# kgnlp/allophant

Measured on AMD Instinct MI355X. Metric: encoder frames/sec (whole node), 10s x 32 utterances @16kHz, higher is better.
Workload: dtype f16x3

## Files before the change

allophant_amd/csrc/amx_api.hip:

```cpp
#include "../../include/allophant_amx.h"
#include "../../include/allophant_amx_allophones.h"
#include "../../include/allophant_amx_beam.h"
#include "../../include/allophant_amx_align.h"
#include "../../include/allophant_amx_score.h"
#include "../../include/allophant_amx_search.h"
#include "../../include/allophant_amx_resample.h"
#include "../../include/allophant_amx_edit.h"
#include "amx_common.h"

#include <algorithm>
#include <cmath>
#include <cstdio>
#include <cstring>
#include <initializer_list>
#include <map>
#include <cstdlib>
#include <string>
#include <vector>

using namespace amx;

namespace {

thread_local std::string g_create_error;
// ... 1106 lines not shown
struct PassPlan {
    uint32_t flags = 0;
    int N = 0;
    int64_t L = 0;
    const float* d_audio = nullptr;
    float* d_out = nullptr;
    int64_t total = 0;
    int NT = 2, prec = 0, C = 0, D = 0, F = 0, H = 0, dh = 64, dhp = 64, E = 0, Eld = 0, cg = 0;
    int64_t Ts[AMX_MAX_CONV + 1] = {};
    int T = 0, Tp = 0, TpTot = 0, Tpad = 0;
    int64_t M = 0, Mp = 0, Mrows = 0, Mh = 0, rows1 = 0, rows2 = 0, xp_plane = 0, qk_plane = 0;
    size_t qkv_bytes = 0;
    bool keep = false, masked = true, stable = true, blanks = true;
    bool packed = false, packed_early = false, ragged = false, window_ok = false, needs_qkv_zero = false;
    bool fold = false, stream_in_planes = false;
    void *d_len = nullptr, *d_frames = nullptr, *d_rowoff = nullptr, *d_partial = nullptr, *d_stats = nullptr, *actA = nullptr, *actB = nullptr,
         *preln = nullptr, *hbuf = nullptr, *xp = nullptr, *hg = nullptr, *qb = nullptr, *kb = nullptr, *vtb = nullptr, *ao = nullptr, *ff = nullptr,
         *hfin = nullptr, *logits = nullptr, *hpk = nullptr, *splitk = nullptr, *gn_partial = nullptr, *gn_scale = nullptr, *gn_shift = nullptr,
         *ebuf = nullptr, *cat = nullptr, *tl_x = nullptr, *tl_p = nullptr, *tl_qkv = nullptr, *ln_rowps = nullptr, *ln_coef = nullptr,
         *ln_partial = nullptr;
    const int* d_frames_enc = nullptr;
    int* d_tiles = nullptr;
    size_t tile_first[AMX_MAX_CONV + 1] = {};
    std::vector<float*> saved;
    float* conv_dbg = nullptr;
    float* hfin_rows = nullptr;
    float* stream = nullptr;
    std::vector<int> rowoff_host, frames_host;

    GemmParams with_ws(GemmParams g) const {
        g.splitk_ws = (float*)splitk;
        g.splitk_ws_elems = splitk ? (int64_t)(SPLITK_BYTES / 4) : 0;
        return g;
    }
    AttnParams attn_params() const {
// ... 37 lines not shown
        return with_ws(g);
    }
    GemmParams ffn2_params(amx_handle h, const Layer& ly) const {
        GemmParams g{};
        g.A = ff; g.a_plane = pln(h, Mrows * F); g.lda = F; g.rows_per_batch = Mrows;
        g.W = ly.w2; g.w_plane = pln(h, (int64_t)D * F); g.ldw = F;
        g.M = (int)Mrows; g.N = D; g.K = F;
        g.scale = ly.r_2; g.bias = ly.b2;
        g.residual = stream; g.ldr = D; g.out_f32 = stream; g.ldo = D;
        return with_ws(g);
    }
    GemmParams as_consumer(GemmParams g, const float* col_c) const {
        g.row_coef = (const float2*)ln_coef; g.col_c = col_c;
        return g;
    }
    GemmParams as_producer(GemmParams g, bool f32 = true) const {
        g.ln_partial = (float2*)ln_partial; g.ln_rowps = (const float4*)ln_rowps;
        g.out_p = xp; g.out_plane = xp_plane; g.ldp = D;
        if (stream_in_planes) {
            g.ln_res_planes = 1;
            g.residual = nullptr;
            if (!f32) g.out_f32 = nullptr;
        }
        return g;
    }
};

}

static int pin_reserve(amx_handle h, int N, hipStream_t s) {
    HIPCHK(h, hipStreamSynchronize(s));
    for (int i = 0; i < amx_handle_s::PIN_SLOTS; ++i) {
// ... 229 lines not shown
    }
    P.blanks = c.dependency_blanks != 0;
    if ((rc = plan_concat(h, P, s))) return rc;
    P.needs_qkv_zero = !P.packed && (h->last_N != N || h->last_T != P.T || h->qkv_dirty);
    P.Mrows = P.packed ? P.Mp : P.M;
    P.xp_plane = pln(h, P.Mrows * D);
    P.qk_plane = P.packed ? (int64_t)H * P.TpTot * P.dhp : (int64_t)N * H * P.Tp * P.dhp;
    P.stream = (float*)(P.packed ? P.hpk : P.hbuf);
    if (P.packed_early) {
        P.rowoff_host.assign(pin_rowoff, pin_rowoff + N);
        P.frames_host.assign(pin_frames, pin_frames + N);
    }
    P.stream_in_planes = NT == 2;
    if (P.stable && c.layers > 0 && D % 64 == 0 && D <= 2048) {
        WS("ln_rowps", (size_t)P.Mrows * 16, P.ln_rowps);
        WS("ln_coef", (size_t)P.Mrows * 8, P.ln_coef);
        WS("ln_partial", (size_t)P.Mrows * (D / 64) * 8, P.ln_partial);
        const Layer& ly = h->layers[0];
        const int prec = P.prec;
        P.fold = gemm_ln_fold_ok(prec, P.as_consumer(P.qkv_params(h, ly), ly.c_qkv)) &&
                 gemm_ln_fold_ok(prec, P.as_producer(P.oproj_params(h, ly), false)) &&
                 gemm_ln_fold_ok(prec, P.as_consumer(P.ffn1_params(h, ly), ly.c_1)) &&
                 gemm_ln_fold_ok(prec, P.as_producer(P.ffn2_params(h, ly), false)) &&
                 gemm_ln_fold_ok(prec, P.as_producer(P.ffn2_params(h, ly), true));
    }
    ++h->pass_counter;
    h->last_fold = P.fold;
    h->last_packed = P.packed_early ? 2 : (P.packed ? 1 : 0);
    h->last_attention = c.layers > 0 ? attention_form(P.attn_params()) : -1;
    h->last_rows = P.Mrows;
    h->last_graph = 0;
#undef WS
    return AMX_OK;
}

static int enqueue_pass(amx_handle h, const PassPlan& P, hipStream_t s) {
    const amx_config& c = h->cfg;
    const int prec = P.prec, N = P.N, C = P.C, D = P.D, T = P.T;
    const int64_t M = P.M, Mh = P.Mh;
// ... 153 lines not shown
            pending.splits = splits;
        }
        gemm(g);
    };
    auto stream_norm = [&](const float* gamma, const float* beta, int64_t rows, int64_t plane, float* out_ln) {
        Timed t_(h, AMX_KC_ROWNORM);
        if (pending.on) {
            launch_fixup_rownorm(prec, pending.g, pending.splits, gamma, beta, c.eps, P.xp, plane, D, out_ln, D, s);
            pending.on = false;
        } else {
            launch_rownorm(prec, (const float*)hbuf, D, rows, D, gamma, beta, 0, nullptr, nullptr, c.eps, 0.f, P.xp, plane, D, out_ln, D, s);
        }
    };
    float* const ln_inplace = P.stable ? nullptr : (float*)hbuf;
    if (!P.stable) stream_norm(h->fln_g, h->fln_b, P.Mrows, P.xp_plane, ln_inplace);
    const int* const fold_frames = P.packed || !P.masked ? nullptr : P.d_frames_enc;
    auto ln_finalize = [&]() {
        Timed t_(h, AMX_KC_ROWNORM);
        launch_ln_finalize((const float2*)P.ln_partial, D / 64, P.Mrows, c.eps, (float4*)P.ln_rowps, (float2*)P.ln_coef, fold_frames, T, s);
    };
    for (int l = 0; l < c.layers; ++l) {
        const Layer& ly = h->layers[l];
        if (P.fold) {
            if (l == 0) {
                Timed t_(h, AMX_KC_ROWNORM);
                launch_ln_rowprep(prec, (const float*)hbuf, D, P.Mrows, D, c.eps, P.xp, P.xp_plane, D, (float4*)P.ln_rowps, (float2*)P.ln_coef,
                                  fold_frames, T, s);
            }
        } else if (P.stable) {
            stream_norm(h->unit_g, h->zero_b, P.Mrows, P.xp_plane, nullptr);
        }
        if (P.saved[l]) {
            if (P.packed_early) {
                launch_copy(P.saved[l], hbuf, (size_t)P.Mp * D * 4, s);
            } else {
                launch_copy(P.saved[l], P.packed ? hpad : hbuf, (size_t)M * D * 4, s);
                if (P.packed) launch_pack_rows(P.saved[l], (float*)hbuf, (const int*)P.d_rowoff, (const int*)P.d_frames, N, T, D, true, s);
            }
        }
        gemm(P.fold ? P.as_consumer(P.qkv_params(h, ly), ly.c_qkv) : P.qkv_params(h, ly));
        {
            Timed t_(h, AMX_KC_ATTENTION);
            launch_attention(prec, P.attn_params(), s);
        }
        if (P.fold) {
            residual_gemm(P.as_producer(P.oproj_params(h, ly), false), false);
            ln_finalize();
        } else {
            residual_gemm(P.oproj_params(h, ly), true);
            if (P.stable) stream_norm(h->unit_g, h->zero_b, P.Mrows, P.xp_plane, nullptr);
            else stream_norm(ly.ln1_g, ly.ln1_b, P.Mrows, P.xp_plane, ln_inplace);
        }
        gemm(P.fold ? P.as_consumer(P.ffn1_params(h, ly), ly.c_1) : P.ffn1_params(h, ly));
        if (P.fold && (l + 1 < c.layers || P.stream_in_planes)) {
            const bool last = l + 1 == c.layers;
            residual_gemm(P.as_producer(P.ffn2_params(h, ly), last || P.saved[l + 1] != nullptr), false);
            if (!last) ln_finalize();
        } else {
            residual_gemm(P.ffn2_params(h, ly), !P.fold && !(P.packed && !P.packed_early && l == c.layers - 1));
        }
        if (!P.stable) stream_norm(ly.ln2_g, ly.ln2_b, P.Mrows, P.xp_plane, ln_inplace);
    }
    if (refused) return fail(h, AMX_EINVAL, "internal: an encoder product of the LayerNorm fold had no kernel for its plan and was not launched");
    if (P.packed && !P.packed_early) {
        { Timed t_(h, AMX_KC_OTHER); launch_pack_rows((const float*)hpad, (float*)P.hpk, (const int*)P.d_rowoff, (const int*)P.d_frames, N, T, D, true, s); }
        hbuf = hpad;
    }
    if (P.stable) {
        stream_norm(h->fln_g, h->fln_b, Mh, pln(h, Mh * D), (float*)P.hfin);
    } else if (P.keep) {
        launch_copy(P.hfin, hbuf, (size_t)Mh * D * 4, s);
    }
// ... 958 lines not shown
```

allophant_amd/csrc/amx_common.h:

```cpp
#pragma once
#include <hip/hip_runtime.h>
#include <stdint.h>
#include <string>
#include <type_traits>

struct amx_resample_geometry;
struct amx_resample_row;

namespace amx {

typedef _Float16 f16;
typedef __bf16 bf16;
typedef __attribute__((ext_vector_type(8))) _Float16 f16x8;
typedef __attribute__((ext_vector_type(8))) __bf16 bf16x8;
typedef __attribute__((ext_vector_type(4))) _Float16 f16x4;
typedef __attribute__((ext_vector_type(4))) __bf16 bf16x4;
typedef __attribute__((ext_vector_type(2))) _Float16 f16x2;
typedef __attribute__((ext_vector_type(2))) __bf16 bf16x2;
typedef __attribute__((ext_vector_type(2))) float f32x2;
typedef __attribute__((ext_vector_type(4))) float f32x4;
typedef __attribute__((ext_vector_type(16))) float f32x16;

enum Precision { PREC_BF16 = 0, PREC_F16 = 1, PREC_BF16X3 = 2, PREC_F16X3 = 3 };
inline int prec_planes(int p) { return p >= 2 ? 2 : 1; }
// ... 200 lines not shown
    float* splitk_ws;
    int64_t splitk_ws_elems;
    int splits;
    int64_t split_out;
    const int* tile_list;
    int n_tiles;
    int defer_fixup;
    int a_taps;
    int64_t a_tap_stride;
    unsigned long long* stamps;
    const float4* ln_rowps;
    float2* ln_partial;
    int ln_res_planes;
    const float2* row_coef;
    const float* col_c;
};

extern bool g_force_generic_gemm;
bool launch_gemm(int prec, const GemmParams& p, hipStream_t stream);
bool gemm_uses_pp(int prec, const GemmParams& p);
bool gemm_fuses_ln(int prec, const GemmParams& p);
int gemm_ln_tap_minor_slice(int prec, const GemmParams& p);
int gemm_planned_splits(int prec, const GemmParams& p);
bool fixup_rownorm_eligible(const GemmParams& p);
void launch_fixup_rownorm(int prec, const GemmParams& p, int splits, const float* gamma, const float* beta, float eps, void* out_p,
                          int64_t out_plane, int64_t ldp, float* out_ln, int64_t ldo_ln, hipStream_t stream);
bool gemm_ln_fold_ok(int prec, const GemmParams& p);
void launch_gemm_grouped(int prec, const GemmParams& p, int groups, hipStream_t stream);

struct AttnParams {
    const void* q;
// ... 217 lines not shown
```

allophant_amd/csrc/amx_gemm.hip:

```cpp
#include "amx_common.h"
#include <algorithm>
#include <cstdlib>
#include <type_traits>

namespace amx {

bool g_force_generic_gemm = false;

namespace {

#include "amx_gemm_tile.inc"
#include "amx_gemm_pp.inc"
#include "amx_gemm_ln.inc"

int device_cus() {
    static int per_device[MAX_DEVICES] = {};
    const int dev = current_device();
    int& cus = per_device[dev];
    if (!cus) {
        hipDeviceProp_t prop;
        if (hipGetDeviceProperties(&prop, dev) == hipSuccess) cus = prop.multiProcessorCount;
        if (cus <= 0) cus = 256;
        cus -= cus % 8;
        if (cus < 8) cus = 8;
// ... 238 lines not shown

enum class GemmKernel { LN, LN_IL, PP, DMA, TILE };

struct GemmRoute {
    GemmKernel kernel = GemmKernel::TILE;
    int mi = 0, ni = 0;
    int fold = 0;
    int shape = 0;
    int bn = 0;
    int splits = 1;
    bool launches = true;
};

GemmRoute gemm_route(int NT, const GemmParams& p) {
    GemmRoute r;
    r.fold = p.ln_partial ? 2 : p.row_coef ? 1 : 0;
    if (p.ln_gamma) {
        r.kernel = ln_uses_il(NT, p) ? GemmKernel::LN_IL : GemmKernel::LN;
        r.launches = ln_eligible(NT, p);
        return r;
    }
    if (!dma_preferred_shape(NT, p) && pp_eligible(NT, p)) {
        r.kernel = GemmKernel::PP;
        pp_plan(NT, p, &r.mi, &r.splits, &r.ni);
        r.launches = !(r.fold == 2 && r.ni != 4);
        return r;
    }
    r.launches = !r.fold;
    r.shape = dma_tile_shape(NT, p, 1);
    if (r.shape) {
        r.kernel = GemmKernel::DMA;
// ... 87 lines not shown
}

static GemmRoute product_route_of(int prec, GemmParams p) {
    p.ln_gamma = nullptr;
    return route_of(prec, p);
}

bool gemm_uses_pp(int prec, const GemmParams& p) { return product_route_of(prec, p).kernel == GemmKernel::PP; }

bool gemm_ln_fold_ok(int prec, const GemmParams& p_in) {
    const GemmParams p = with_vec_flag(p_in);
    const int NT = prec_planes(prec);
    const GemmRoute r = product_route_of(prec, p_in);
    if (!p.vec_ok || r.kernel != GemmKernel::PP || r.splits != 1) return false;
    if (p.ln_partial) {
        if (r.ni != 4 || p.N % 64 || p.N > 2048 || !p.out_p || !p.ln_rowps || p.act || p.mode || p.row_len || p.row_coef) return false;
        if (p.ln_res_planes ? NT != 2 : (!p.out_f32 || !p.residual)) return false;
        if (NT == 2 && (p.out_plane != PLANE_IL || p.ldp % 32)) return false;
        if (p.ldp % 8 || ((uintptr_t)p.out_p & 15) || ((uintptr_t)p.ln_partial & 7) || ((uintptr_t)p.ln_rowps & 15)) return false;
    }
    if (p.row_coef) {
        if (!p.col_c || ((uintptr_t)p.col_c & 15) || ((uintptr_t)p.row_coef & 7) || p.residual || p.row_len) return false;
        if (p.mode != 1 && (!p.out_p || p.out_f32)) return false;
    }
    return true;
}

int gemm_planned_splits(int prec, const GemmParams& p) { return route_of(prec, p).splits; }

bool fixup_rownorm_eligible(const GemmParams& p) {
    return p.splitk_ws && p.out_f32 && !p.out_p && p.act == 0 && p.mode == 0 && !p.row_len && !p.ln_gamma && p.N % 4 == 0 &&
           p.N <= 1024 && p.ldo % 4 == 0 && (!p.residual || p.ldr % 4 == 0) && !((uintptr_t)p.out_f32 & 15) &&
           !((uintptr_t)p.residual & 15) && !((uintptr_t)p.bias & 15) && p.zout == 0;
}

void launch_fixup_rownorm(int prec, const GemmParams& p, int splits, const float* gamma, const float* beta, float eps, void* out_p,
                          int64_t out_plane, int64_t ldp, float* out_ln, int64_t ldo_ln, hipStream_t stream) {
    AMX_DISPATCH(prec, (launch_fixup_rownorm_t<T16, NT>(p, splits, gamma, beta, eps, out_p, out_plane, ldp, out_ln, ldo_ln, stream)));
// ... 17 lines not shown
```

allophant_amd/csrc/amx_gemm_pp.inc:

```

namespace pp {
constexpr int BN = 256;
constexpr int EPI_WAVE = 32 * 64 * 4;
template <int MI, int NI = 4>
struct Ring {
    static constexpr int A_BYTES = MI * 32 * 128, W_BYTES = NI * 64 * 128, SLICE = A_BYTES + W_BYTES;
    static constexpr int NSL = MI == 8 ? 2 : 3, DIST = NSL - 1;
    static constexpr int EPI_BASE = DIST * SLICE;
    static constexpr int LDS_BYTES = (NSL * SLICE > EPI_BASE + 8 * EPI_WAVE) ? NSL * SLICE : EPI_BASE + 8 * EPI_WAVE;
};
constexpr int lds_bytes(int NT, int MI, int NI = 4) {
    return MI == 8 ? (NI == 4 ? Ring<8, 4>::LDS_BYTES : Ring<8, 3>::LDS_BYTES) : (NI == 4 ? Ring<4, 4>::LDS_BYTES : Ring<4, 3>::LDS_BYTES);
}
constexpr int epi_base(int NT, int MI, int NI = 4) {
    return MI == 8 ? (NI == 4 ? Ring<8, 4>::EPI_BASE : Ring<8, 3>::EPI_BASE) : (NI == 4 ? Ring<4, 4>::EPI_BASE : Ring<4, 3>::EPI_BASE);
}
__device__ __forceinline__ int es_idx(int row, int chunk) { return row * 64 + ((chunk ^ (row & 7)) << 2); }
}

__device__ __forceinline__ void mfma16_acc(f32x4& c, f16x8 a, f16x8 b) {
    asm volatile("v_mfma_f32_16x16x32_f16 %0, %1, %2, %0" : "+v"(c) : "v"(a), "v"(b));
}
__device__ __forceinline__ void mfma16_acc(f32x4& c, bf16x8 a, bf16x8 b) {
    asm volatile("v_mfma_f32_16x16x32_bf16 %0, %1, %2, %0" : "+v"(c) : "v"(a), "v"(b));
// ... 151 lines not shown
            const float4 pr = ps[j % SLOTS][i];
            float4 v = make_float4(fmaf(c[i][0], scale, b4.x), fmaf(c[i][1], scale, b4.y), fmaf(c[i][2], scale, b4.z),
                                   fmaf(c[i][3], scale, b4.w));
            float4 res = r[j % SLOTS][i];
            if (RESP) {
                const uint4 raw = __builtin_bit_cast(uint4, res);
                res = pp_planes_residual<T>(make_uint2(raw.x, raw.y), make_uint2(raw.z, raw.w), pr.x, pow2_reciprocal(pr.y));
            }
            v.x += res.x; v.y += res.y; v.z += res.z; v.w += res.w;
            if (optr) *(float4*)(optr + (int64_t)row * p.ldo) = v;
            pp_emit_row<T, NT>(v, make_float2(pr.z, pr.w), ch, true, part + (int64_t)row * nblk, pbase + (int64_t)row * prow, plane);
        }
    }
}

template <typename T, int NT, bool ACT, bool QK, int MI, bool FINISHED = false, int NI = 4, bool COEF = false>
__device__ __forceinline__ void pp_epilogue_p16(const GemmParams& p, f32x4 (&acc)[NI][MI], float* es, int lane, int mw, int nw) {
    typedef typename Vec8<T>::type V8;
    const int c8 = NI == 4 || (lane & 7) < 2 * NI ? (lane & 7) : (lane & 7) - 2 * NI, rs = lane >> 3;
    const int n = nw + c8 * 8;
    const float scale = FINISHED ? 1.f : p.scale;
    float4 b0 = make_float4(0.f, 0.f, 0.f, 0.f), b1 = b0;
    if (!FINISHED && p.bias) { b0 = *(const float4*)(p.bias + n); b1 = *(const float4*)(p.bias + n + 4); }
    float4 cc0 = make_float4(0.f, 0.f, 0.f, 0.f), cc1 = cc0;
    if (COEF) { cc0 = *(const float4*)(p.col_c + n); cc1 = *(const float4*)(p.col_c + n + 4); }
    const float2* coef = COEF ? p.row_coef + (mw + rs) : nullptr;
    T* base;
    int64_t row_stride, plane;
    int b = 0, t = 0;
    if (QK) {
        const int D = p.H * p.dh;
        const int which = n / D;
        const int rem = n - which * D;
        const int hh = rem / p.dh, d = rem - hh * p.dh;
        base = (T*)(which == 0 ? p.q : (which == 1 ? p.k : p.v)) + (int64_t)hh * p.Tp * p.dhp + d;
        row_stride = p.dhp;
        plane = p.qk_plane;
        b = (mw + rs) / p.T;
        t = (mw + rs) - b * p.T;
    } else {
        const bool o_il = plane_is_il<NT>(p.out_plane);
        base = (T*)p.out_p + pidx((int64_t)(mw + rs) * p.ldp + n, o_il);
        row_stride = p.ldp << (o_il ? 1 : 0);
        plane = p.out_plane;
    }
    float2 cf_all[MI / 2][4];
    if (COEF) {
#pragma unroll
        for (int q = 0; q < MI / 2; ++q)
#pragma unroll
            for (int i = 0; i < 4; ++i) cf_all[q][i] = coef[q * 32 + i * 8];
    }
#pragma unroll
    for (int q = 0; q < MI / 2; ++q) {
        float2 cf[4];
        if (COEF) {
#pragma unroll
            for (int i = 0; i < 4; ++i) cf[i] = cf_all[q][i];
        }
        pp_stage_round(es, acc, q, lane);
        f32x4 c[4][2];
#pragma unroll
        for (int i = 0; i < 4; ++i) {
            c[i][0] = *(const f32x4*)(es + pp::es_idx(i * 8 + rs, 2 * c8));
            c[i][1] = *(const f32x4*)(es + pp::es_idx(i * 8 + rs, 2 * c8 + 1));
        }
#pragma unroll
        for (int i = 0; i < 4; ++i) {
            float v[8];
            if (COEF) {
                const float as = cf[i].x * scale, bs = cf[i].y;
                v[0] = fmaf(c[i][0][0], as, fmaf(bs, cc0.x, b0.x)); v[1] = fmaf(c[i][0][1], as, fmaf(bs, cc0.y, b0.y));
                v[2] = fmaf(c[i][0][2], as, fmaf(bs, cc0.z, b0.z)); v[3] = fmaf(c[i][0][3], as, fmaf(bs, cc0.w, b0.w));
// ... 18 lines not shown
                t += 8;
                const bool wrap = t >= p.T;
                t -= wrap ? p.T : 0;
                b += wrap ? 1 : 0;
            } else {
                dst = base + (int64_t)(q * 32 + i * 8) * row_stride;
            }
            *(V8*)dst = hv.v;
            if (NT > 1) *(V8*)(dst + plane) = lv.v;
        }
    }
}

template <typename T, int NT, int MI, bool FINISHED = false, int NI = 4, int FOLD = 0>
__device__ __forceinline__ void pp_epilogue_generic(const GemmParams& p, f32x4 (&acc)[NI][MI], float* es, int lane, int mw, int nw,
                                                    float* out_f32) {
    typedef typename Vec4<T>::type V4;
    const int D = p.H * p.dh;
    const float scale = FINISHED ? 1.f : p.scale;
    const int ch = lane & 15, rq = (lane >> 4) * 8;
    const int n = nw + ch * 4;
    const bool n_ok = n < p.N && ch < NI * 4;
    float4 bias4 = make_float4(0.f, 0.f, 0.f, 0.f);
    if (!FINISHED && p.bias && n_ok) bias4 = *(const float4*)(p.bias + n);
    int64_t qk_col = 0;
    T* qk_base = nullptr;
    if (p.mode == 1 && n_ok) {
        const int which = n / D;
        const int rem = n - which * D;
        const int hh = rem / p.dh, d = rem - hh * p.dh;
        qk_base = (T*)(which == 0 ? p.q : (which == 1 ? p.k : p.v));
// ... 5 lines not shown
    if (FOLD == 1 && n_ok) colc4 = *(const float4*)(p.col_c + n);
    constexpr bool emit = NI == 4 && FOLD == 2;
#pragma unroll
    for (int q = 0; q < MI / 2; ++q) {
        pp_stage_round(es, acc, q, lane);
        int b = 0, t = 0;
        if (need_bt) {
            const int mfirst = mw + q * 32 + rq;
            b = mfirst / rt;
            t = mfirst - b * rt;
        }
#pragma unroll
        for (int i = 0; i < 8; ++i) {
            const int m = mw + q * 32 + rq + i;
            const f32x4 c = *(const f32x4*)(es + pp::es_idx(rq + i, ch));
            if constexpr (emit) {
                const bool ok = m < p.M;
                const int mc = ok ? m : p.M - 1;
                float4 v = make_float4(fmaf(c[0], scale, bias4.x), fmaf(c[1], scale, bias4.y), fmaf(c[2], scale, bias4.z),
                                       fmaf(c[3], scale, bias4.w));
                const float4 pr = p.ln_rowps[mc];
                T* pdst = (T*)p.out_p + pidx((int64_t)mc * p.ldp + n, NT == 2);
                const int64_t plane = NT == 2 ? PLANE_IL : 0;
                float4 rr = make_float4(0.f, 0.f, 0.f, 0.f);
                if constexpr (NT == 2) {
                    if (p.ln_res_planes) rr = pp_planes_residual<T>(*(const uint2*)pdst, *(const uint2*)(pdst + plane), pr.x, pow2_reciprocal(pr.y));
                    else if (p.residual) rr = *(const float4*)(p.residual + (int64_t)mc * p.ldr + n);
                } else if (p.residual) {
                    rr = *(const float4*)(p.residual + (int64_t)mc * p.ldr + n);
                }
                v.x += rr.x; v.y += rr.y; v.z += rr.z; v.w += rr.w;
                if (ok && out_f32) *(float4*)(out_f32 + (int64_t)m * p.ldo + n) = v;
                pp_emit_row<T, NT>(v, make_float2(pr.z, pr.w), ch, ok, p.ln_partial + (int64_t)mc * (p.N >> 6) + (n >> 6), pdst, plane);
                continue;
            }
            if (m < p.M && n_ok) {
                float v[4];
                if (FOLD == 1) {
                    const float2 cf = p.row_coef[m];
                    const float as = cf.x * scale;
                    v[0] = fmaf(c[0], as, fmaf(cf.y, colc4.x, bias4.x)); v[1] = fmaf(c[1], as, fmaf(cf.y, colc4.y, bias4.y));
                    v[2] = fmaf(c[2], as, fmaf(cf.y, colc4.z, bias4.z)); v[3] = fmaf(c[3], as, fmaf(cf.y, colc4.w, bias4.w));
                } else {
                    v[0] = fmaf(c[0], scale, bias4.x); v[1] = fmaf(c[1], scale, bias4.y);
                    v[2] = fmaf(c[2], scale, bias4.z); v[3] = fmaf(c[3], scale, bias4.w);
                }
                if (!FINISHED && p.act == 1) {
#pragma unroll
                    for (int r = 0; r < 4; r += 2) {
                        const f32x2 g = gelu_fast2(f32x2{v[r], v[r + 1]});
                        v[r] = g[0];
                        v[r + 1] = g[1];
                    }
                }
// ... 268 lines not shown
        const int mw = m0 + grp * HALF, nw = n0 + wc * (16 * NI);
        float* out_f32 = p.out_f32 ? p.out_f32 + (int64_t)ks * p.split_out : nullptr;
        const int next = it + gridDim.x;
        const bool has_next = next < total;
        if (has_next) {
            setup_tile(next);
            stage_head();
        }

#ifndef AMX_ABLATE_NO_EPI
        asm volatile("" : "+v"(lane));
        if (nw < p.N && mw < p.M) {
            float* es = (float*)(smem + pp::epi_base(NT, MI, NI) + wave * pp::EPI_WAVE);
            bool done = false;
            if constexpr (FOLD == 1) {
                if (mw + HALF <= p.M && nw + 16 * NI <= p.N && p.vec_ok) {
                    if (p.mode == 1) {
                        if (p.T >= 8 && p.dh % 8 == 0 && p.qk_plane % 8 == 0 && !(((uintptr_t)p.q | (uintptr_t)p.k | (uintptr_t)p.v) & 15)) {
                            pp_epilogue_p16<T, NT, false, true, MI, false, NI, true>(p, acc, es, lane, mw, nw);
                            done = true;
                        }
                    } else if (p.out_p && !p.out_f32 && p.ldp % 8 == 0 && p.out_plane % 8 == 0 && !((uintptr_t)p.out_p & 15)) {
                        if (p.act == 1) pp_epilogue_p16<T, NT, true, false, MI, false, NI, true>(p, acc, es, lane, mw, nw);
                        else pp_epilogue_p16<T, NT, false, false, MI, false, NI, true>(p, acc, es, lane, mw, nw);
                        done = true;
                    }
                }
                if (!done) pp_epilogue_generic<T, NT, MI, false, NI, 1>(p, acc, es, lane, mw, nw, out_f32);
            } else if constexpr (FOLD == 2) {
                if constexpr (NI == 4) {
                    if (mw + HALF <= p.M && nw + 16 * NI <= p.N && p.vec_ok) {
                        if constexpr (NT == 2) {
                            if (p.ln_res_planes) pp_epilogue_f32_emit<T, NT, MI, true>(p, acc, es, lane, mw, nw, out_f32);
                            else pp_epilogue_f32_emit<T, NT, MI, false>(p, acc, es, lane, mw, nw, out_f32);
                        } else {
                            pp_epilogue_f32_emit<T, NT, MI, false>(p, acc, es, lane, mw, nw, out_f32);
                        }
                    } else {
                        pp_epilogue_generic<T, NT, MI, false, NI, 2>(p, acc, es, lane, mw, nw, out_f32);
                    }
                }
            } else {
            if (mw + HALF <= p.M && nw + 16 * NI <= p.N && !p.row_len && p.vec_ok) {
// ... 44 lines not shown
```

allophant_amd/csrc/amx_rowops.hip:

```cpp
#include "amx_common.h"
#include <cstdlib>

namespace amx {

namespace {

constexpr int STAT_CHUNKS = 64;

__global__ __launch_bounds__(256) void audio_stats_kernel(const float* __restrict__ audio, const int64_t* __restrict__ lengths,
                                                          int64_t L, double* __restrict__ partial) {
    const int n = blockIdx.y, c = blockIdx.x;
    int64_t per = (L + STAT_CHUNKS - 1) / STAT_CHUNKS;
    per = (per + 3) & ~(int64_t)3;
    int64_t lo = c * per, hi = lo + per < L ? lo + per : L;
    const int64_t len = lengths[n];
    const float* row = audio + (int64_t)n * L;
    double s_all = 0, s_val = 0, q_val = 0;
    for (int64_t i = lo + threadIdx.x; i < hi; i += 256) {
        double x = row[i];
        s_all += x;
        if (i < len) { s_val += x; q_val += x * x; }
    }
    __shared__ double red[3][4];
#pragma unroll
// ... 787 lines not shown
                split16<T, NT>(v[i].z, hi[2], lo[2]);
                split16<T, NT>(v[i].w, hi[3], lo[3]);
                T* dst = out_p + pidx(row * ldp + c, plane_is_il<NT>(out_plane));
                typedef typename Vec4<T>::type V4;
                V4 hv = {hi[0], hi[1], hi[2], hi[3]};
                *(V4*)dst = hv;
                if (NT > 1) {
                    V4 lv = {lo[0], lo[1], lo[2], lo[3]};
                    *(V4*)(dst + out_plane) = lv;
                }
            }
        }
    }
}

constexpr float LN_PAD_SCALE = 0x1p-6f;
__device__ __forceinline__ float ln_plane_scale(float rstd, bool padded) {
    const float t = fminf(fmaxf(2.0f * rstd, 1.0e-12f), 1.0e12f);
    const float s = __uint_as_float(__float_as_uint(t) & 0x7F800000u);
    return padded ? s * LN_PAD_SCALE : s;
}
__device__ __forceinline__ bool ln_padded_row(int64_t row, const int* frame_len, int T_rows) {
    return frame_len && (int)(row % T_rows) >= frame_len[row / T_rows];
}

template <typename T, int NT, int V = 4>
__global__ __launch_bounds__(256) void ln_rowprep_kernel(const float* __restrict__ x, int64_t ldx, int64_t M, int D, float eps,
                                                         T* __restrict__ out_p, int64_t out_plane, int64_t ldp,
                                                         float4* __restrict__ rowps, float2* __restrict__ coef,
                                                         const int* __restrict__ frame_len, int T_rows) {
    const int lane = threadIdx.x & 63;
    const int64_t row = (int64_t)blockIdx.x * 4 + (threadIdx.x >> 6);
    if (row >= M) return;
    const float* src = x + row * ldx;
    float4 v[V];
    const float invD = 1.0f / (float)D;
#pragma unroll
    for (int i = 0; i < V; ++i) {
        const int c = (i * 64 + lane) * 4;
        v[i] = c < D ? *(const float4*)(src + c) : make_float4(0.f, 0.f, 0.f, 0.f);
// ... 32 lines not shown
            *(V4*)dst = hv;
            if (NT > 1) {
                V4 lv = {lo[0], lo[1], lo[2], lo[3]};
                *(V4*)(dst + out_plane) = lv;
            }
        }
    }
}

__global__ __launch_bounds__(256) void ln_finalize_kernel(const float2* __restrict__ partial, int blocks, int64_t M, float eps,
                                                          float4* __restrict__ rowps, float2* __restrict__ coef,
                                                          const int* __restrict__ frame_len, int T_rows) {
    const int64_t row = (int64_t)blockIdx.x * 256 + threadIdx.x;
    if (row >= M) return;
    const float2* pr = partial + row * blocks;
    float2 b[32];
    float s1 = 0.f;
#pragma unroll
    for (int j = 0; j < 32; ++j)
        if (j < blocks) {
            b[j] = pr[j];
            s1 += b[j].x;
        }
    const float4 ps = rowps[row];
    const float inv_w = __uint_as_float(0x7F000000u - __float_as_uint(ps.w));
    const float invD = 1.0f / (float)(blocks * 64);
    const float mu = s1 * invD;
    float m2 = 0.f;
#pragma unroll
    for (int j = 0; j < 32; ++j)
        if (j < blocks) {
            const float d = b[j].x * (1.0f / 64.0f) - mu;
            m2 += fmaf(64.0f * d, d, b[j].y);
        }
    const float m1 = mu * inv_w;
    const float rs = 1.0f / sqrtf(m2 * invD * inv_w * inv_w + eps);
    coef[row] = make_float2(rs * inv_w, -rs * m1);
    rowps[row] = make_float4(ps.z, ps.w, ps.z + m1, ln_plane_scale(rs, ln_padded_row(row, frame_len, T_rows)));
}

template <typename T, int NT>
__global__ __launch_bounds__(256) void posconv_pack_kernel(const float* __restrict__ h, int N, int Tn, int D, int G,
                                                           int pad_front, int Tpad, T* __restrict__ out, int64_t out_plane,
                                                           const int* __restrict__ row_off, const int* __restrict__ frame_len) {
    const int cg = D / G;
    const int64_t total4 = (int64_t)G * N * Tpad * cg / 4;
    for (int64_t i = (int64_t)blockIdx.x * 256 + threadIdx.x; i < total4; i += (int64_t)gridDim.x * 256) {
        int64_t e = i * 4;
        int ci = (int)(e % cg);
        int64_t r = e / cg;
        int tp = (int)(r % Tpad);
        r /= Tpad;
        int n = (int)(r % N);
// ... 763 lines not shown
```

Before: 548,400.

## Fuse layernorm finalize into consumer GEMM epilogue with ping-pong row stats

Removes the standalone ln_finalize kernel launched after the o-proj and FFN2 GEMMs. The consumer GEMMs (QKV for layers after the first, and FFN1) now merge the per-block partial statistics themselves in their epilogue, producing the row coefficients in registers and sharing them across lanes with ds_bpermute. Row stats move through two alternating buffers so that a reader and a writer never touch the same array. This saves two launches and two global round-trips per layer, but every N-tile of the consumer GEMM recomputes the merge redundantly and the epilogue gains register and LDS pressure.

```diff
diff --git a/allophant_amd/csrc/amx_api.hip b/allophant_amd/csrc/amx_api.hip
--- a/allophant_amd/csrc/amx_api.hip
+++ b/allophant_amd/csrc/amx_api.hip
@@ -1144,11 +1144,13 @@
     bool keep = false, masked = true, stable = true, blanks = true;
     bool packed = false, packed_early = false, ragged = false, window_ok = false, needs_qkv_zero = false;
     bool fold = false, stream_in_planes = false;
+    const int* fold_frames = nullptr;
+    float eps = 0.f;
     void *d_len = nullptr, *d_frames = nullptr, *d_rowoff = nullptr, *d_partial = nullptr, *d_stats = nullptr, *actA = nullptr, *actB = nullptr,
          *preln = nullptr, *hbuf = nullptr, *xp = nullptr, *hg = nullptr, *qb = nullptr, *kb = nullptr, *vtb = nullptr, *ao = nullptr, *ff = nullptr,
          *hfin = nullptr, *logits = nullptr, *hpk = nullptr, *splitk = nullptr, *gn_partial = nullptr, *gn_scale = nullptr, *gn_shift = nullptr,
-         *ebuf = nullptr, *cat = nullptr, *tl_x = nullptr, *tl_p = nullptr, *tl_qkv = nullptr, *ln_rowps = nullptr, *ln_coef = nullptr,
-         *ln_partial = nullptr;
+         *ebuf = nullptr, *cat = nullptr, *tl_x = nullptr, *tl_p = nullptr, *tl_qkv = nullptr, *ln_rowps = nullptr, *ln_rowps_b = nullptr,
+         *ln_coef = nullptr, *ln_partial = nullptr;
     const int* d_frames_enc = nullptr;
     int* d_tiles = nullptr;
     size_t tile_first[AMX_MAX_CONV + 1] = {};
@@ -1216,8 +1218,21 @@
         g.row_coef = (const float2*)ln_coef; g.col_c = col_c;
         return g;
     }
-    GemmParams as_producer(GemmParams g, bool f32 = true) const {
-        g.ln_partial = (float2*)ln_partial; g.ln_rowps = (const float4*)ln_rowps;
+    const float4* rowps_array(int which) const { return (const float4*)(which ? ln_rowps_b : ln_rowps); }
+    GemmParams as_merging_consumer(GemmParams g, const float* col_c, int from) const {
+        g.col_c = col_c;
+        g.ln_merge_partial = (const float2*)ln_partial; g.ln_merge_blocks = D / 64;
+        g.ln_rowps_in = rowps_array(from); g.ln_rowps_out = (float4*)rowps_array(from ^ 1);
+        g.ln_merge_eps = eps;
+        g.ln_frame_len = fold_frames; g.ln_rows_T = T;
+        return g;
+    }
+    GemmParams fold_qkv(amx_handle h, const Layer& ly, int l) const {
+        return l == 0 ? as_consumer(qkv_params(h, ly), ly.c_qkv) : as_merging_consumer(qkv_params(h, ly), ly.c_qkv, 1);
+    }
+    GemmParams fold_ffn1(amx_handle h, const Layer& ly) const { return as_merging_consumer(ffn1_params(h, ly), ly.c_1, 0); }
+    GemmParams as_producer(GemmParams g, bool f32, int pairs) const {
+        g.ln_partial = (float2*)ln_partial; g.ln_rowps = rowps_array(pairs);
         g.out_p = xp; g.out_plane = xp_plane; g.ldp = D;
         if (stream_in_planes) {
             g.ln_res_planes = 1;
@@ -1477,15 +1492,18 @@
     P.stream_in_planes = NT == 2;
     if (P.stable && c.layers > 0 && D % 64 == 0 && D <= 2048) {
         WS("ln_rowps", (size_t)P.Mrows * 16, P.ln_rowps);
+        WS("ln_rowps_b", (size_t)P.Mrows * 16, P.ln_rowps_b);
         WS("ln_coef", (size_t)P.Mrows * 8, P.ln_coef);
         WS("ln_partial", (size_t)P.Mrows * (D / 64) * 8, P.ln_partial);
+        P.fold_frames = P.packed || !P.masked ? nullptr : P.d_frames_enc;
+        P.eps = c.eps;
         const Layer& ly = h->layers[0];
         const int prec = P.prec;
-        P.fold = gemm_ln_fold_ok(prec, P.as_consumer(P.qkv_params(h, ly), ly.c_qkv)) &&
-                 gemm_ln_fold_ok(prec, P.as_producer(P.oproj_params(h, ly), false)) &&
-                 gemm_ln_fold_ok(prec, P.as_consumer(P.ffn1_params(h, ly), ly.c_1)) &&
-                 gemm_ln_fold_ok(prec, P.as_producer(P.ffn2_params(h, ly), false)) &&
-                 gemm_ln_fold_ok(prec, P.as_producer(P.ffn2_params(h, ly), true));
+        P.fold = gemm_ln_fold_ok(prec, P.fold_qkv(h, ly, 0)) && gemm_ln_fold_ok(prec, P.fold_qkv(h, ly, 1)) &&
+                 gemm_ln_fold_ok(prec, P.as_producer(P.oproj_params(h, ly), false, 0)) &&
+                 gemm_ln_fold_ok(prec, P.fold_ffn1(h, ly)) &&
+                 gemm_ln_fold_ok(prec, P.as_producer(P.ffn2_params(h, ly), false, 1)) &&
+                 gemm_ln_fold_ok(prec, P.as_producer(P.ffn2_params(h, ly), true, 1));
     }
     ++h->pass_counter;
     h->last_fold = P.fold;
@@ -1669,18 +1687,13 @@
     };
     float* const ln_inplace = P.stable ? nullptr : (float*)hbuf;
     if (!P.stable) stream_norm(h->fln_g, h->fln_b, P.Mrows, P.xp_plane, ln_inplace);
-    const int* const fold_frames = P.packed || !P.masked ? nullptr : P.d_frames_enc;
-    auto ln_finalize = [&]() {
-        Timed t_(h, AMX_KC_ROWNORM);
-        launch_ln_finalize((const float2*)P.ln_partial, D / 64, P.Mrows, c.eps, (float4*)P.ln_rowps, (float2*)P.ln_coef, fold_frames, T, s);
-    };
     for (int l = 0; l < c.layers; ++l) {
         const Layer& ly = h->layers[l];
         if (P.fold) {
             if (l == 0) {
                 Timed t_(h, AMX_KC_ROWNORM);
                 launch_ln_rowprep(prec, (const float*)hbuf, D, P.Mrows, D, c.eps, P.xp, P.xp_plane, D, (float4*)P.ln_rowps, (float2*)P.ln_coef,
-                                  fold_frames, T, s);
+                                  P.fold_frames, T, s);
             }
         } else if (P.stable) {
             stream_norm(h->unit_g, h->zero_b, P.Mrows, P.xp_plane, nullptr);
@@ -1693,24 +1706,22 @@
                 if (P.packed) launch_pack_rows(P.saved[l], (float*)hbuf, (const int*)P.d_rowoff, (const int*)P.d_frames, N, T, D, true, s);
             }
         }
-        gemm(P.fold ? P.as_consumer(P.qkv_params(h, ly), ly.c_qkv) : P.qkv_params(h, ly));
+        gemm(P.fold ? P.fold_qkv(h, ly, l) : P.qkv_params(h, ly));
         {
             Timed t_(h, AMX_KC_ATTENTION);
             launch_attention(prec, P.attn_params(), s);
         }
         if (P.fold) {
-            residual_gemm(P.as_producer(P.oproj_params(h, ly), false), false);
-            ln_finalize();
+            residual_gemm(P.as_producer(P.oproj_params(h, ly), false, 0), false);
         } else {
             residual_gemm(P.oproj_params(h, ly), true);
             if (P.stable) stream_norm(h->unit_g, h->zero_b, P.Mrows, P.xp_plane, nullptr);
             else stream_norm(ly.ln1_g, ly.ln1_b, P.Mrows, P.xp_plane, ln_inplace);
         }
-        gemm(P.fold ? P.as_consumer(P.ffn1_params(h, ly), ly.c_1) : P.ffn1_params(h, ly));
+        gemm(P.fold ? P.fold_ffn1(h, ly) : P.ffn1_params(h, ly));
         if (P.fold && (l + 1 < c.layers || P.stream_in_planes)) {
             const bool last = l + 1 == c.layers;
-            residual_gemm(P.as_producer(P.ffn2_params(h, ly), last || P.saved[l + 1] != nullptr), false);
-            if (!last) ln_finalize();
+            residual_gemm(P.as_producer(P.ffn2_params(h, ly), last || P.saved[l + 1] != nullptr, 1), false);
         } else {
             residual_gemm(P.ffn2_params(h, ly), !P.fold && !(P.packed && !P.packed_early && l == c.layers - 1));
         }
diff --git a/allophant_amd/csrc/amx_common.h b/allophant_amd/csrc/amx_common.h
--- a/allophant_amd/csrc/amx_common.h
+++ b/allophant_amd/csrc/amx_common.h
@@ -238,7 +238,50 @@
     int ln_res_planes;
     const float2* row_coef;
     const float* col_c;
-};
+    const float2* ln_merge_partial;
+    int ln_merge_blocks;
+    const float4* ln_rowps_in;
+    float4* ln_rowps_out;
+    float ln_merge_eps;
+    const int* ln_frame_len;
+    int ln_rows_T;
+};
+
+#ifdef __HIPCC__
+constexpr float LN_PAD_SCALE = 0x1p-6f;
+constexpr int LN_MAX_BLOCKS = 32;
+__device__ __forceinline__ float ln_plane_scale(float rstd, bool padded) {
+    const float t = fminf(fmaxf(2.0f * rstd, 1.0e-12f), 1.0e12f);
+    const float s = __uint_as_float(__float_as_uint(t) & 0x7F800000u);
+    return padded ? s * LN_PAD_SCALE : s;
+}
+__device__ __forceinline__ bool ln_padded_row(int64_t row, const int* frame_len, int T_rows) {
+    return frame_len && (int)(row % T_rows) >= frame_len[row / T_rows];
+}
+template <int NB>
+__device__ __forceinline__ void ln_merge_row(const float2 (&b)[NB], int blocks, float4 ps, float eps, bool padded, float2& coef,
+                                             float4& next) {
+#pragma clang fp contract(off)
+    float s1 = 0.f;
+#pragma unroll
+    for (int j = 0; j < NB; ++j)
+        if (j < blocks) s1 += b[j].x;
+    const float inv_w = __uint_as_float(0x7F000000u - __float_as_uint(ps.w));
+    const float invD = 1.0f / (float)(blocks * 64);
+    const float mu = s1 * invD;
+    float m2 = 0.f;
+#pragma unroll
+    for (int j = 0; j < NB; ++j)
+        if (j < blocks) {
+            const float d = b[j].x * (1.0f / 64.0f) - mu;
+            m2 += fmaf(64.0f * d, d, b[j].y);
+        }
+    const float m1 = mu * inv_w;
+    const float rs = 1.0f / sqrtf(m2 * invD * inv_w * inv_w + eps);
+    coef = make_float2(rs * inv_w, -rs * m1);
+    next = make_float4(ps.z, ps.w, ps.z + m1, ln_plane_scale(rs, padded));
+}
+#endif
 
 extern bool g_force_generic_gemm;
 bool launch_gemm(int prec, const GemmParams& p, hipStream_t stream);
diff --git a/allophant_amd/csrc/amx_gemm.hip b/allophant_amd/csrc/amx_gemm.hip
--- a/allophant_amd/csrc/amx_gemm.hip
+++ b/allophant_amd/csrc/amx_gemm.hip
@@ -276,7 +276,7 @@
 
 GemmRoute gemm_route(int NT, const GemmParams& p) {
     GemmRoute r;
-    r.fold = p.ln_partial ? 2 : p.row_coef ? 1 : 0;
+    r.fold = p.ln_partial ? 2 : (p.row_coef || p.ln_merge_partial) ? 1 : 0;
     if (p.ln_gamma) {
         r.kernel = ln_uses_il(NT, p) ? GemmKernel::LN_IL : GemmKernel::LN;
         r.launches = ln_eligible(NT, p);
@@ -394,14 +394,21 @@
     const GemmRoute r = product_route_of(prec, p_in);
     if (!p.vec_ok || r.kernel != GemmKernel::PP || r.splits != 1) return false;
     if (p.ln_partial) {
-        if (r.ni != 4 || p.N % 64 || p.N > 2048 || !p.out_p || !p.ln_rowps || p.act || p.mode || p.row_len || p.row_coef) return false;
+        if (r.ni != 4 || p.N % 64 || p.N > 2048 || !p.out_p || !p.ln_rowps || p.act || p.mode || p.row_len || p.row_coef || p.ln_merge_partial)
+            return false;
         if (p.ln_res_planes ? NT != 2 : (!p.out_f32 || !p.residual)) return false;
         if (NT == 2 && (p.out_plane != PLANE_IL || p.ldp % 32)) return false;
         if (p.ldp % 8 || ((uintptr_t)p.out_p & 15) || ((uintptr_t)p.ln_partial & 7) || ((uintptr_t)p.ln_rowps & 15)) return false;
     }
-    if (p.row_coef) {
+    if (p.row_coef || p.ln_merge_partial) {
         if (!p.col_c || ((uintptr_t)p.col_c & 15) || ((uintptr_t)p.row_coef & 7) || p.residual || p.row_len) return false;
         if (p.mode != 1 && (!p.out_p || p.out_f32)) return false;
+    }
+    if (p.ln_merge_partial) {
+        if (p.row_coef || p.ln_merge_blocks < 1 || p.ln_merge_blocks > LN_MAX_BLOCKS || (int64_t)p.ln_merge_blocks * 64 != p.K) return false;
+        if (!p.ln_rowps_in || !p.ln_rowps_out || (const float4*)p.ln_rowps_out == p.ln_rowps_in) return false;
+        if (((uintptr_t)p.ln_merge_partial & 7) || ((uintptr_t)p.ln_rowps_in & 15) || ((uintptr_t)p.ln_rowps_out & 15)) return false;
+        if (p.ln_frame_len && (p.ln_rows_T < 1 || ((uintptr_t)p.ln_frame_len & 3))) return false;
     }
     return true;
 }
diff --git a/allophant_amd/csrc/amx_gemm_pp.inc b/allophant_amd/csrc/amx_gemm_pp.inc
--- a/allophant_amd/csrc/amx_gemm_pp.inc
+++ b/allophant_amd/csrc/amx_gemm_pp.inc
@@ -189,8 +189,125 @@
     }
 }
 
+template <int RPL>
+struct MergedCoef {
+    float2 v[RPL];
+};
+template <int RPL, int NB, int ALL>
+__device__ __forceinline__ void pp_merge_rows(const GemmParams& p, int lane, int mw, int r0, bool store, MergedCoef<ALL>& own) {
+    constexpr int SLOTS = NB ? NB : LN_MAX_BLOCKS;
+    const int blocks = NB ? NB : p.ln_merge_blocks;
+    float2 b[RPL][SLOTS];
+    float4 ps[RPL];
+    int row[RPL], flen[RPL], frame[RPL];
+#pragma unroll
+    for (int r = 0; r < RPL; ++r) {
+        row[r] = mw + (r0 + r) * 64 + lane;
+        const int rc = row[r] < p.M ? row[r] : p.M - 1;
+        const float2* pr = p.ln_merge_partial + (int64_t)rc * blocks;
+#pragma unroll
+        for (int j = 0; j < SLOTS; ++j)
+            if (NB || j < blocks) b[r][j] = pr[j];
+        ps[r] = p.ln_rowps_in[rc];
+        flen[r] = 0x7fffffff;
+        frame[r] = 0;
+        if (p.ln_frame_len) {
+            const int u = rc / p.ln_rows_T;
+            frame[r] = rc - u * p.ln_rows_T;
+            flen[r] = p.ln_frame_len[u];
+        }
+    }
+#pragma unroll
+    for (int r = 0; r < RPL; ++r) {
+        float4 next;
+        ln_merge_row(b[r], blocks, ps[r], p.ln_merge_eps, frame[r] >= flen[r], own.v[r0 + r], next);
+        if (store && row[r] < p.M) p.ln_rowps_out[row[r]] = next;
+    }
+}
+template <int RPL, int NB>
+__device__ __forceinline__ void pp_merge_rows_lds(const GemmParams& p, float* es, int lane, int mw, bool store, MergedCoef<RPL>& own) {
+    static_assert(NB <= 16, "64 rows of statistics must fit the epilogue patch");
+    f32x2* cs = (f32x2*)es;
+    const f32x2* src = (const f32x2*)p.ln_merge_partial;
+    const int last = p.M * NB - 1;
+    f32x2 raw[RPL][NB];
+    float4 ps[RPL];
+    int row[RPL], flen[RPL], frame[RPL];
+#pragma unroll
+    for (int r = 0; r < RPL; ++r) {
+        const int base = (mw + r * 64) * NB + lane;
+#pragma unroll
+        for (int i = 0; i < NB; ++i) {
+            const int e = base + i * 64;
+            raw[r][i] = src[e < last ? e : last];
+        }
+        row[r] = mw + r * 64 + lane;
+        const int rc = row[r] < p.M ? row[r] : p.M - 1;
+        ps[r] = p.ln_rowps_in[rc];
+        flen[r] = 0x7fffffff;
+        frame[r] = 0;
+        if (p.ln_frame_len) {
+            const int u = rc / p.ln_rows_T;
+            frame[r] = rc - u * p.ln_rows_T;
+            flen[r] = p.ln_frame_len[u];
+        }
+    }
+    const int lm = lane % NB;
+#pragma unroll
+    for (int r = 0; r < RPL; ++r) {
+#pragma unroll
+        for (int i = 0; i < NB; ++i) {
+            const int e = i * 64 + lane, rw = e / NB, j = e - rw * NB;
+            int c = j + rw % NB;
+            c -= c >= NB ? NB : 0;
+            cs[rw * NB + c] = raw[r][i];
+        }
+        float2 b[NB];
+#pragma unroll
+        for (int j = 0; j < NB; ++j) {
+            int c = j + lm;
+            c -= c >= NB ? NB : 0;
+            const f32x2 v = cs[lane * NB + c];
+            b[j] = make_float2(v[0], v[1]);
+        }
+        float4 next;
+        ln_merge_row(b, NB, ps[r], p.ln_merge_eps, frame[r] >= flen[r], own.v[r], next);
+        if (store && row[r] < p.M) p.ln_rowps_out[row[r]] = next;
+    }
+}
+template <int MI>
+__device__ __forceinline__ void pp_merge_coef(const GemmParams& p, float* es, int lane, int mw, int nw, MergedCoef<MI / 4>& own) {
+    constexpr int RPL = MI / 4;
+    const bool store = nw == 0;
+    switch (p.ln_merge_blocks) {
+        case 16: pp_merge_rows_lds<RPL, 16>(p, es, lane, mw, store, own); break;
+        case 12: pp_merge_rows_lds<RPL, 12>(p, es, lane, mw, store, own); break;
+        default:
+#pragma unroll
+            for (int r = 0; r < RPL; ++r) {
+                if (p.ln_merge_blocks == 20) pp_merge_rows<1, 20, RPL>(p, lane, mw, r, store, own);
+                else if (p.ln_merge_blocks == 30) pp_merge_rows<1, 30, RPL>(p, lane, mw, r, store, own);
+                else pp_merge_rows<1, 0, RPL>(p, lane, mw, r, store, own);
+            }
+    }
+}
+template <int MI>
+__device__ __forceinline__ void pp_load_coef(const GemmParams& p, int lane, int mw, MergedCoef<MI / 4>& own) {
+#pragma unroll
+    for (int r = 0; r < MI / 4; ++r) {
+        const int row = mw + r * 64 + lane;
+        own.v[r] = p.row_coef[row < p.M ? row : p.M - 1];
+    }
+}
+template <int RPL>
+__device__ __forceinline__ float2 pp_merged_coef(const MergedCoef<RPL>& own, int reg, int src_lane) {
+    return make_float2(__builtin_bit_cast(float, __builtin_amdgcn_ds_bpermute(src_lane << 2, __builtin_bit_cast(int, own.v[reg].x))),
+                       __builtin_bit_cast(float, __builtin_amdgcn_ds_bpermute(src_lane << 2, __builtin_bit_cast(int, own.v[reg].y))));
+}
+
 template <typename T, int NT, bool ACT, bool QK, int MI, bool FINISHED = false, int NI = 4, bool COEF = false>
-__device__ __forceinline__ void pp_epilogue_p16(const GemmParams& p, f32x4 (&acc)[NI][MI], float* es, int lane, int mw, int nw) {
+__device__ __forceinline__ void pp_epilogue_p16(const GemmParams& p, f32x4 (&acc)[NI][MI], float* es, int lane, int mw, int nw,
+                                                const MergedCoef<MI / 4>& own = MergedCoef<MI / 4>{}) {
     typedef typename Vec8<T>::type V8;
     const int c8 = NI == 4 || (lane & 7) < 2 * NI ? (lane & 7) : (lane & 7) - 2 * NI, rs = lane >> 3;
     const int n = nw + c8 * 8;
@@ -199,7 +316,6 @@
     if (!FINISHED && p.bias) { b0 = *(const float4*)(p.bias + n); b1 = *(const float4*)(p.bias + n + 4); }
     float4 cc0 = make_float4(0.f, 0.f, 0.f, 0.f), cc1 = cc0;
     if (COEF) { cc0 = *(const float4*)(p.col_c + n); cc1 = *(const float4*)(p.col_c + n + 4); }
-    const float2* coef = COEF ? p.row_coef + (mw + rs) : nullptr;
     T* base;
     int64_t row_stride, plane;
     int b = 0, t = 0;
@@ -219,19 +335,12 @@
         row_stride = p.ldp << (o_il ? 1 : 0);
         plane = p.out_plane;
     }
-    float2 cf_all[MI / 2][4];
-    if (COEF) {
-#pragma unroll
-        for (int q = 0; q < MI / 2; ++q)
-#pragma unroll
-            for (int i = 0; i < 4; ++i) cf_all[q][i] = coef[q * 32 + i * 8];
-    }
 #pragma unroll
     for (int q = 0; q < MI / 2; ++q) {
         float2 cf[4];
         if (COEF) {
 #pragma unroll
-            for (int i = 0; i < 4; ++i) cf[i] = cf_all[q][i];
+            for (int i = 0; i < 4; ++i) cf[i] = pp_merged_coef(own, q >> 1, (q & 1) * 32 + i * 8 + rs);
         }
         pp_stage_round(es, acc, q, lane);
         f32x4 c[4][2];
@@ -280,7 +389,7 @@
 
 template <typename T, int NT, int MI, bool FINISHED = false, int NI = 4, int FOLD = 0>
 __device__ __forceinline__ void pp_epilogue_generic(const GemmParams& p, f32x4 (&acc)[NI][MI], float* es, int lane, int mw, int nw,
-                                                    float* out_f32) {
+                                                    float* out_f32, const MergedCoef<MI / 4>& own = MergedCoef<MI / 4>{}) {
     typedef typename Vec4<T>::type V4;
     const int D = p.H * p.dh;
     const float scale = FINISHED ? 1.f : p.scale;
@@ -316,6 +425,8 @@
         for (int i = 0; i < 8; ++i) {
             const int m = mw + q * 32 + rq + i;
             const f32x4 c = *(const f32x4*)(es + pp::es_idx(rq + i, ch));
+            float2 mcf = make_float2(0.f, 0.f);
+            if (FOLD == 1) mcf = pp_merged_coef(own, q >> 1, (q & 1) * 32 + rq + i);
             if constexpr (emit) {
                 const bool ok = m < p.M;
                 const int mc = ok ? m : p.M - 1;
@@ -339,7 +450,7 @@
             if (m < p.M && n_ok) {
                 float v[4];
                 if (FOLD == 1) {
-                    const float2 cf = p.row_coef[m];
+                    const float2 cf = mcf;
                     const float as = cf.x * scale;
                     v[0] = fmaf(c[0], as, fmaf(cf.y, colc4.x, bias4.x)); v[1] = fmaf(c[1], as, fmaf(cf.y, colc4.y, bias4.y));
                     v[2] = fmaf(c[2], as, fmaf(cf.y, colc4.z, bias4.z)); v[3] = fmaf(c[3], as, fmaf(cf.y, colc4.w, bias4.w));
@@ -638,19 +749,22 @@
             float* es = (float*)(smem + pp::epi_base(NT, MI, NI) + wave * pp::EPI_WAVE);
             bool done = false;
             if constexpr (FOLD == 1) {
+                MergedCoef<MI / 4> own;
+                if (p.ln_merge_partial) pp_merge_coef<MI>(p, es, lane, mw, nw, own);
+                else pp_load_coef<MI>(p, lane, mw, own);
                 if (mw + HALF <= p.M && nw + 16 * NI <= p.N && p.vec_ok) {
                     if (p.mode == 1) {
                         if (p.T >= 8 && p.dh % 8 == 0 && p.qk_plane % 8 == 0 && !(((uintptr_t)p.q | (uintptr_t)p.k | (uintptr_t)p.v) & 15)) {
-                            pp_epilogue_p16<T, NT, false, true, MI, false, NI, true>(p, acc, es, lane, mw, nw);
+                            pp_epilogue_p16<T, NT, false, true, MI, false, NI, true>(p, acc, es, lane, mw, nw, own);
                             done = true;
                         }
                     } else if (p.out_p && !p.out_f32 && p.ldp % 8 == 0 && p.out_plane % 8 == 0 && !((uintptr_t)p.out_p & 15)) {
-                        if (p.act == 1) pp_epilogue_p16<T, NT, true, false, MI, false, NI, true>(p, acc, es, lane, mw, nw);
-                        else pp_epilogue_p16<T, NT, false, false, MI, false, NI, true>(p, acc, es, lane, mw, nw);
+                        if (p.act == 1) pp_epilogue_p16<T, NT, true, false, MI, false, NI, true>(p, acc, es, lane, mw, nw, own);
+                        else pp_epilogue_p16<T, NT, false, false, MI, false, NI, true>(p, acc, es, lane, mw, nw, own);
                         done = true;
                     }
                 }
-                if (!done) pp_epilogue_generic<T, NT, MI, false, NI, 1>(p, acc, es, lane, mw, nw, out_f32);
+                if (!done) pp_epilogue_generic<T, NT, MI, false, NI, 1>(p, acc, es, lane, mw, nw, out_f32, own);
             } else if constexpr (FOLD == 2) {
                 if constexpr (NI == 4) {
                     if (mw + HALF <= p.M && nw + 16 * NI <= p.N && p.vec_ok) {
diff --git a/allophant_amd/csrc/amx_rowops.hip b/allophant_amd/csrc/amx_rowops.hip
--- a/allophant_amd/csrc/amx_rowops.hip
+++ b/allophant_amd/csrc/amx_rowops.hip
@@ -825,16 +825,6 @@
     }
 }
 
-constexpr float LN_PAD_SCALE = 0x1p-6f;
-__device__ __forceinline__ float ln_plane_scale(float rstd, bool padded) {
-    const float t = fminf(fmaxf(2.0f * rstd, 1.0e-12f), 1.0e12f);
-    const float s = __uint_as_float(__float_as_uint(t) & 0x7F800000u);
-    return padded ? s * LN_PAD_SCALE : s;
-}
-__device__ __forceinline__ bool ln_padded_row(int64_t row, const int* frame_len, int T_rows) {
-    return frame_len && (int)(row % T_rows) >= frame_len[row / T_rows];
-}
-
 template <typename T, int NT, int V = 4>
 __global__ __launch_bounds__(256) void ln_rowprep_kernel(const float* __restrict__ x, int64_t ldx, int64_t M, int D, float eps,
                                                          T* __restrict__ out_p, int64_t out_plane, int64_t ldp,
@@ -897,29 +887,15 @@
     const int64_t row = (int64_t)blockIdx.x * 256 + threadIdx.x;
     if (row >= M) return;
     const float2* pr = partial + row * blocks;
-    float2 b[32];
-    float s1 = 0.f;
-#pragma unroll
-    for (int j = 0; j < 32; ++j)
-        if (j < blocks) {
-            b[j] = pr[j];
-            s1 += b[j].x;
-        }
-    const float4 ps = rowps[row];
-    const float inv_w = __uint_as_float(0x7F000000u - __float_as_uint(ps.w));
-    const float invD = 1.0f / (float)(blocks * 64);
-    const float mu = s1 * invD;
-    float m2 = 0.f;
-#pragma unroll
-    for (int j = 0; j < 32; ++j)
-        if (j < blocks) {
-            const float d = b[j].x * (1.0f / 64.0f) - mu;
-            m2 += fmaf(64.0f * d, d, b[j].y);
-        }
-    const float m1 = mu * inv_w;
-    const float rs = 1.0f / sqrtf(m2 * invD * inv_w * inv_w + eps);
-    coef[row] = make_float2(rs * inv_w, -rs * m1);
-    rowps[row] = make_float4(ps.z, ps.w, ps.z + m1, ln_plane_scale(rs, ln_padded_row(row, frame_len, T_rows)));
+    float2 b[LN_MAX_BLOCKS];
+#pragma unroll
+    for (int j = 0; j < LN_MAX_BLOCKS; ++j)
+        if (j < blocks) b[j] = pr[j];
+    float2 cf;
+    float4 next;
+    ln_merge_row(b, blocks, rowps[row], eps, ln_padded_row(row, frame_len, T_rows), cf, next);
+    coef[row] = cf;
+    rowps[row] = next;
 }
 
 template <typename T, int NT>
```

Result: slower. 537,000 (-2.1%).
